# google/data-driven-discretization-1d

Hardware: AMD Instinct MI355X
Metric: grid-point-steps/s (higher is better)
Workload: dtype f32

## Files before the change

data-driven-discretization-1d_amd/csrc/capi.hip:

```cpp
#include <hip/hip_runtime.h>

#include <emmintrin.h>

#include <algorithm>
#include <chrono>
#include <cmath>
#include <condition_variable>
#include <cstdarg>
#include <cstdio>
#include <cstdlib>
#include <cstring>
#include <mutex>
#include <string>
#include <thread>
#include <type_traits>
#include <vector>

#include "../../include/ddd1d.h"
#include "dev_params.h"
#include "launch.h"
#include "launch_weno.h"
#include "ops.h"
#include "pack_weights.h"
#ifdef DDD_PROBES
// ... 235 lines not shown
  const char* name = nullptr;
};

}

struct ddd_model {
  ddd_config cfg;
  ddd::DevParams dp;
  bool mfma_ok = false;
  std::string mfma_reason;
  int kernel = DDD_KERNEL_GENERIC;
  int force_rows = 0;
  bool explicit_kernel = false;
  bool spec_folded = false;
  Plan last_plan;
  int64_t fma_per_point = 0;
  float* d_weights = nullptr;
  float* d_weights4 = nullptr;
  float* d_nullspace = nullptr;
  float* d_bias = nullptr;
  float* d_w_input = nullptr;
  float* d_w_hidden = nullptr;
  float* d_w_final4 = nullptr;
  float* d_w_final4_rt = nullptr;
  float* d_w_final4_split = nullptr;
  float* d_w_quad = nullptr;
  float* d_w_final4_half = nullptr;
  float* d_w_t16 = nullptr;
  bool wide = false;
  int tower_k = 5, tower_cb = 1;
  bool big() const { return tower_k != ddd::mfma::kKW || tower_cb != 1; }
  float4* d_frc = nullptr;
  float* d_sp = nullptr;
  float* d_trig = nullptr;
  unsigned char* d_runs = nullptr;
  bool spectral = false;
  ddd::spectral::Params sp{};
  double* d_kernels = nullptr;
  double2* d_fft_mult = nullptr;
  double2* d_fft_twiddle = nullptr;
  double* d_scratch64 = nullptr;
  size_t scratch64_doubles = 0;
  hipStream_t aux_stream[4] = {nullptr, nullptr, nullptr, nullptr};
  hipEvent_t ev_fork = nullptr, ev_join[4] = {nullptr, nullptr, nullptr, nullptr};
  struct Chain {
    bool open = false;
// ... 114 lines not shown
  in.wide = m->wide; in.tower_k = m->tower_k; in.tower_cb = m->tower_cb;
  in.no_fold = g_debug.no_fold != 0;
  in.net = net;
  const ddd::pack::Packed packed = ddd::pack::pack_weights(in);
  int rc = upload(packed.w_input, &m->d_w_input);
  if (!rc) rc = upload(packed.w_hidden, &m->d_w_hidden);
  if (!rc && packed.unsupported) rc = DDD_ERR_UNSUPPORTED;
  if (!rc) rc = upload(packed.w_final4_rt, &m->d_w_final4_rt);
  if (!rc) rc = upload(packed.w_final4, &m->d_w_final4);
  if (!rc) rc = upload(packed.w_final4_split, &m->d_w_final4_split);
  if (!rc) rc = upload(packed.w_quad, &m->d_w_quad);
  if (!rc) rc = upload(packed.w_final4_half, &m->d_w_final4_half);
  if (!rc) rc = upload(packed.w_t16, &m->d_w_t16);
  dp.w_input = m->d_w_input;
  dp.w_hidden = m->d_w_hidden;
  dp.w_final4_rt = m->d_w_final4_rt;
  dp.w_final4 = m->d_w_final4;
  dp.w_final4_split = m->d_w_final4_split;
  dp.w_quad = m->d_w_quad;
  dp.folded = packed.folded;
  dp.rt_groups = packed.rt_groups;
  dp.fin4_groups = packed.fin4_groups;
  m->spec_folded = packed.spec_folded;
  return rc;
}

bool linear_eligible(const ddd::DevParams& dp) {
  return !dp.fixed && dp.L == 1 && dp.target == ddd::TARGET_COEFFICIENTS &&
         !(dp.pao <= 0 && dp.unbiased) && dp.D <= 3 && dp.G <= ddd::kGMax && dp.K <= 7 &&
         dp.K * dp.D <= ddd::kChMax;
}

void decide_mfma(ddd_model* m) {
  const ddd::DevParams& dp = m->dp;
  char why[256] = "";
  bool ok = true;
  auto no = [&](const char* msg) { if (ok) snprintf(why, sizeof(why), "%s", msg); ok = false; };
  if (dp.N < 8 || dp.N > 256) no("num_points outside [8, 256]");
  if (dp.G > ddd::kGWide) no("stencil wider than 12");
  if (dp.G > dp.N) no("stencil wider than the grid");
  if (dp.fixed && dp.weno) no("WENO reconstruction");
  bool wide = dp.G > ddd::kGMax;
  const bool linear = linear_eligible(dp);
  if (!dp.fixed && !linear) {
    if (dp.target == ddd::TARGET_COEFFICIENTS && dp.pao <= 0 && dp.D > 2) wide = true;
    if (dp.C_out > ddd::kChMax) wide = true;
// ... 104 lines not shown

int spec_equation(const ddd_model* m, int rows) {
  const ddd::DevParams& dp = m->dp;
  if (g_debug.no_spec || m->wide || m->big()) return -1;
  if (dp.forced) {
    const int spg = rows / dp.N;
    const bool fast = spg * dp.P <= rows && dp.n_k <= 6 &&
                      spg * ddd::mfma::kTrigMax <= 3 * rows / 4 && dp.P < 256;
    if (!fast) return -1;
  }
  if (dp.fixed || dp.L != 3 || dp.act != ddd::ACT_RELU) return -1;
  if (dp.target != ddd::TARGET_COEFFICIENTS || dp.pao <= 0) return -1;
  if (dp.equation < ddd::EQ_BURGERS || dp.equation > ddd::EQ_KS_CONS) return -1;
  if (dp.D != ddd::mfma::spec_derivs(dp.equation)) return -1;
  if (dp.G != ddd::mfma::spec_stencil(dp.equation)) return -1;
  if ((dp.conservative != 0) != ddd::mfma::spec_flux_form(dp.equation)) return -1;
  int start = 0;
  for (int d = 0; d < dp.D; ++d) {
    if (dp.in_size[d] != ddd::mfma::spec_in_size(dp.equation, d) || dp.in_start[d] != start)
      return -1;
    start += dp.in_size[d];
  }
  if (m->spec_folded != ddd::mfma::spec_folded(dp.equation)) return -1;
  return dp.equation;
}

bool aligned16(const void* ptr) {
  return (reinterpret_cast<uintptr_t>(ptr) & 15u) == 0;
}

bool use_weno_kernel(const ddd_model* m) {
  return m->kernel == DDD_KERNEL_GENERIC && !m->explicit_kernel && !g_debug.no_weno &&
         ddd::weno::supports(m->dp);
}

template <int kK, int kD, typename F>
bool lean_kernel_if(int taps, int derivs, F& f) {
  if (taps != kK || derivs != kD) return false;
  f(std::integral_constant<int, kK>{}, std::integral_constant<int, kD>{});
  return true;
}
template <typename F>
bool with_lean_kernel(const ddd::DevParams& dp, F&& f) {
  if (!ddd::lean::supports(dp)) return false;
  const int t = dp.fixed ? 0 : dp.linear_taps, d = dp.D;
  return lean_kernel_if<0, 1>(t, d, f) || lean_kernel_if<0, 2>(t, d, f) ||
// ... 2238 lines not shown
    DDD_HIP(hipMalloc(reinterpret_cast<void**>(&d_in), 128 * sizeof(float)));
    DDD_HIP(hipMalloc(reinterpret_cast<void**>(&d_out), 192 * sizeof(float)));
    DDD_HIP(hipMemcpy(d_in, h_in.data(), 128 * sizeof(float), hipMemcpyHostToDevice));
    hipLaunchKernelGGL(ddd::ops::relu_clamp_probe_kernel, dim3(1), dim3(64), 0, nullptr, d_in, d_out);
    DDD_HIP(hipGetLastError());
    std::vector<float> h_out(192);
    DDD_HIP(hipMemcpy(h_out.data(), d_out, 192 * sizeof(float), hipMemcpyDeviceToHost));
    (void)hipFree(d_in);
    (void)hipFree(d_out);
    for (int l = 0; l < 64; ++l)
      for (int e = 0; e < 2; ++e) {
        const float x = h_in[2 * l + e], got = h_out[64 * e + l];
        const float want = std::isnan(x) ? 0.0f : x < 0.0f ? 0.0f : x > 1.0f ? 1.0f : x;
        if (!(got == want) || std::signbit(got))
          return fail(DDD_ERR_UNSUPPORTED,
                      "v_pk_add_f32 ... clamp is not the [0, 1] clamp the relu assumes: "
                      "input %g (element %d of pair %d) gave %g, want %g", x, e, l, got, want);
      }
    for (int l = 0; l < 64; ++l)
      if (h_out[128 + l] != (l < 32 ? (float)l : 1.0f))
        return fail(DDD_ERR_UNSUPPORTED, "constant-lane-mask select: lane %d gave %g", l,
                    h_out[128 + l]);
  }
  (void)dpp_wave_rol_ok();
  return DDD_OK;
}

}
```

data-driven-discretization-1d_amd/csrc/mfma_layout.h:

```cpp
#pragma once

#if defined(__HIP__) || defined(__HIPCC__)
#define DDD_HD __host__ __device__
#else
#define DDD_HD
#endif

namespace ddd {

constexpr int kMaxLayers = 8;
constexpr int kGMax = 8;
constexpr int kGWide = 12;
constexpr int kChMax = 16, kChWide = 24;

constexpr int kReluShift = 64;

enum : int { ACT_NONE = -1, ACT_RELU = 0, ACT_RELU6 = 1, ACT_TANH = 2,
             ACT_SOFTPLUS = 3, ACT_ELU = 4 };
enum : int { TARGET_COEFFICIENTS = 0, TARGET_SPACE_DERIVATIVES = 1,
             TARGET_TIME_DERIVATIVE = 2, TARGET_FLUX = 3 };

namespace mfma {

constexpr int kF = 32;
constexpr int kKW = 5;
constexpr int kInSteps = 3;
constexpr int kHidSteps = 81;
constexpr int kFin4K = kKW * kF + 1;
DDD_HD constexpr int flavour_stencil(bool wide) { return wide ? kGWide : kGMax; }
DDD_HD constexpr int flavour_channels(bool wide) { return wide ? kChWide : kChMax; }
constexpr int kWideDerivs = 3;
DDD_HD constexpr int flavour_net_channels(bool wide) {
  return wide ? kWideDerivs * kGWide : kChMax;
}
DDD_HD constexpr int wide_slot(int G) { return G <= kGMax ? kGMax : G; }

constexpr int kT16InSteps = 2, kT16HidSteps = 4 * kKW + 1;

DDD_HD constexpr int fin4_regs(int groups) { return (kFin4K * groups + 15) / 16; }
DDD_HD constexpr int rt_head_groups(int groups) {
  return groups % 2 == 0 ? 0 : groups == 1 ? 1 : 3;
}

constexpr int padded_rows4(int rows) { return (rows + 3) / 4 * 4; }

constexpr int kQuadHidSteps = 41, kQuadFinSteps = 41, kQuadInSteps = 2;
constexpr int kQuadRows = 2 * kQuadInSteps + 2 * kQuadHidSteps + kQuadFinSteps;

}
}
```

data-driven-discretization-1d_amd/csrc/ops.h:

```cpp
#pragma once
#include "dev_params.h"

namespace ddd {
namespace ops {

__global__ void conv1d_periodic_kernel(const float* __restrict__ in,
                                       const float* __restrict__ w,
                                       const float* __restrict__ bias,
                                       float* __restrict__ out, int batch, int n,
                                       int cin, int cout, int k, int left, int act) {
  const long total = (long)batch * n * cout;
  for (long idx = blockIdx.x * (long)blockDim.x + threadIdx.x; idx < total;
       idx += (long)gridDim.x * blockDim.x) {
    const int co = (int)(idx % cout);
    const long bx = idx / cout;
    const int x = (int)(bx % n);
    const long b = bx / n;
    float acc = 0.0f;
    for (int kk = 0; kk < k; ++kk) {
      int src = (x + kk - left) % n;
      src = src < 0 ? src + n : src;
      const float* row = in + ((size_t)b * n + src) * cin;
      const float* wk = w + (size_t)kk * cin * cout + co;
      for (int ci = 0; ci < cin; ++ci) acc = fmaf(row[ci], wk[(size_t)ci * cout], acc);
// ... 127 lines not shown
  }
}

template <int kAbid>
__device__ __forceinline__ f32x4 mfma4_bcast(float a, float b, f32x4 c) {
  return __builtin_amdgcn_mfma_f32_4x4x1f32(a, b, c, 4, kAbid, 0);
}

__global__ void mfma4_layout_probe_kernel(float* __restrict__ out) {
  const int l = threadIdx.x;
  const float a = (float)(1000 * (l >> 2) + (l & 3) + 1);
  const float b = (float)(l + 1);
#define DDD_P4(ABID)                                                        \
  {                                                                         \
    f32x4 acc = {0.5f, 0.5f, 0.5f, 0.5f};                                   \
    acc = mfma4_bcast<ABID>(a, b, acc);                                     \
    for (int r = 0; r < 4; ++r) out[(ABID * 4 + r) * 64 + l] = acc[r];      \
  }
  DDD_P4(0) DDD_P4(1) DDD_P4(2) DDD_P4(3) DDD_P4(4) DDD_P4(5) DDD_P4(6) DDD_P4(7)
  DDD_P4(8) DDD_P4(9) DDD_P4(10) DDD_P4(11) DDD_P4(12) DDD_P4(13) DDD_P4(14) DDD_P4(15)
#undef DDD_P4
}

__global__ void relu_clamp_probe_kernel(const float* __restrict__ in, float* __restrict__ out) {
  typedef float f32x2 __attribute__((ext_vector_type(2)));
  const int l = threadIdx.x;
  f32x2 v{in[2 * l], in[2 * l + 1]}, y;
  asm volatile("v_pk_add_f32 %0, %1, 0 clamp" : "=v"(y) : "v"(v));
  out[l] = y[0];
  out[64 + l] = y[1];
  float sel;
  const float x = (float)l;
  asm volatile("v_cndmask_b32_e64 %0, %1, 1.0, %2" : "=v"(sel) : "v"(x), "s"(0xffffffff00000000ull));
  out[128 + l] = sel;
}

}
}
```

data-driven-discretization-1d_amd/csrc/pack_weights.h:

```cpp
#pragma once
#include <cmath>
#include <cstddef>
#include <vector>

#include "mfma_layout.h"

namespace ddd {
namespace pack {

struct NetLayout {
  const float* weights;
  int w_off[kMaxLayers], b_off[kMaxLayers];
};

struct Input {
  int L, D, G, C_out, cout0, act, target, pao;
  const int* in_start;
  const int* in_size;
  const float (*ns8)[kGWide];
  const float (*bias8)[kGWide];
  bool wide;
  int tower_k, tower_cb;
  bool no_fold;
  NetLayout net;
};

struct Packed {
  std::vector<float> w_input, w_hidden, w_final4_rt, w_final4, w_final4_split, w_quad,
      w_final4_half, w_t16;
  int folded = 0, rt_groups = 0, fin4_groups = 0;
  bool spec_folded = false;
  bool unsupported = false;
};

inline std::vector<float> quad_rows(const float* rows64, int rows) {
  std::vector<float> out((size_t)ddd::mfma::padded_rows4(rows) * 64, 0.0f);
  for (int s = 0; s < rows; ++s)
    for (int lane = 0; lane < 64; ++lane)
      out[((size_t)(s >> 2) * 64 + lane) * 4 + (s & 3)] = rows64[(size_t)s * 64 + lane];
  return out;
}

template <class Params>
void embed_tower(const Params& dp, const std::vector<float>& wv, int tower_k,
                 int tower_c, std::vector<float>* padded, NetLayout* net) {
  const int k5 = tower_k, f32 = tower_c;
  const int shift = (k5 - 1) / 2 - dp.K / 2;
  padded->clear();
  for (int l = 0; l < dp.L; ++l) {
    const int cin = l == 0 ? 1 : f32;
    const int cout = l == dp.L - 1 ? dp.C_out : f32;
    net->w_off[l] = (int)padded->size();
// ... 112 lines not shown
        acc += (double)b_nat[start + j] * (double)in.ns8[start + j][g];
      f.b[oc] = (float)acc;
    }
  return f;
}

inline int natural_row(int k) { return k; }
inline int tile16_row(int k) { return (k / 16) * 32 + k % 16; }

inline void pack_groups4(const OutLayer& src, float up, int kc, int (*src_row)(int),
                         int first_group, int ng, float* rows) {
  for (int k = 0; k <= kc; ++k)
    for (int gi = 0; gi < ng; ++gi) {
      const int q = k * ng + gi;
      for (int r = 0; r < 4; ++r) {
        const int ch = 4 * (first_group + gi) + r;
        if (ch >= src.live) continue;
        rows[(size_t)(q / 16) * 64 + 4 * (q % 16) + r] =
            k < kc ? up * src.w[(size_t)src_row(k) * src.cols + ch] : src.b[ch];
      }
    }
}

inline std::vector<float> pack_final4_rt(const OutLayer& src, float up, int kc, int groups) {
  const auto regs = [kc](int ng) { return ((kc + 1) * ng + 15) / 16; };
  const int head = mfma::rt_head_groups(groups);
  const int total_rows = regs(head) + (groups - head) / 2 * regs(2) + regs(3);
  std::vector<float> packed((size_t)total_rows * 64, 0.0f);
  if (head > 0) pack_groups4(src, up, kc, natural_row, 0, head, packed.data());
  for (int g0 = head; g0 < groups; g0 += 2)
    pack_groups4(src, up, kc, natural_row, g0, 2,
                 packed.data() + (size_t)(regs(head) + (g0 - head) / 2 * regs(2)) * 64);
  return packed;
}


inline void pack_input16(const float* w0, const float* b0, float dn, int c0, float* rows) {
  for (int lane = 0; lane < 64; ++lane) {
    const int sg = lane >> 4, cout = c0 + (lane & 15);
    rows[lane] = dn * w0[sg * 32 + cout];
    rows[64 + lane] = sg == 0 ? dn * w0[4 * 32 + cout] : sg == 1 ? dn * b0[cout] : 0.0f;
  }
}

inline std::vector<float> pack_quad(const float* w0, const float* b0, const float* w1,
                                    const float* b1, const OutLayer& src, float dn, float up) {
// ... 63 lines not shown
    }
  }

  const float* w_nat = w(in.L - 1);
  const float* b_nat = b(in.L - 1);
  const Fold fold = fold_output_layer(in, w_nat, b_nat, kc);
  const OutLayer plain{w_nat, b_nat, in.C_out, in.C_out};

  const auto issue_cost = [](int groups) { return groups == 1 ? 13.2 : 8.1 * groups; };
  const int groups_plain = (in.C_out + 3) / 4;
  const int groups_rt_folded = ((in.D - 1) * fold.slot + in.G + 3) / 4;
  const bool fold_rt = fold.can_fold && (fold.always || issue_cost(groups_rt_folded) <=
                                                            issue_cost(groups_plain) + 2.5);
  if (fold.wide && !fold_rt) {
    out.unsupported = true;
    return out;
  }
  out.folded = fold_rt ? 1 : 0;
  out.rt_groups = fold_rt ? groups_rt_folded : groups_plain;
  const OutLayer folded_rt{fold.w.data(), fold.b.data(), fold.cols, fold.cols};
  out.w_final4_rt = pack_final4_rt(fold_rt ? folded_rt : plain, up, kc, out.rt_groups);

  const int groups_folded = (in.D * in.G + 3) / 4;
  out.spec_folded = fold.can_fold && groups_folded <= groups_plain;
  out.fin4_groups = out.spec_folded ? groups_folded : groups_plain;
  if (in.wide || big || out.fin4_groups > 4) return out;
  const OutLayer folded_spec{fold.w.data(), fold.b.data(), fold.cols, in.D * in.G};
  const OutLayer& spec = out.spec_folded ? folded_spec : plain;
  const int groups = out.fin4_groups, rows4 = mfma::fin4_regs(4), kc5 = mfma::kFin4K - 1;
  {
    std::vector<float> rows((size_t)rows4 * 64, 0.0f);
    pack_groups4(spec, up, kc5, natural_row, 0, groups, rows.data());
    out.w_final4 = quad_rows(rows.data(), rows4);
  }
  const int na = (groups + 1) / 2, chunk_rows = mfma::fin4_regs(2);
  for (int c = 0; c < 2; ++c) {
    std::vector<float> chunk((size_t)chunk_rows * 64, 0.0f);
    pack_groups4(spec, up, kc5, natural_row, c == 0 ? 0 : na, c == 0 ? na : groups - na,
                 chunk.data());
    const std::vector<float> q4 = quad_rows(chunk.data(), chunk_rows);
    out.w_final4_split.insert(out.w_final4_split.end(), q4.begin(), q4.end());
  }
  if (in.L != 3) return out;
  out.w_quad = pack_quad(w(0), b(0), w(1), b(1), spec, dn, up);
  if (in.cout0 <= 16) {
    std::vector<float> rows((size_t)rows4 * 64, 0.0f);
    pack_groups4(spec, up, 80, tile16_row, 0, groups, rows.data());
    out.w_final4_half = quad_rows(rows.data(), rows4);
    out.w_t16 = pack_t16(w(0), b(0), w(1), b(1), dn);
  }
  return out;
}

}
}
```

data-driven-discretization-1d_amd/csrc/rhs_adaptive.h:

```cpp
#pragma once
#include "rhs_mfma.h"
#include "rk23.h"
#ifdef DDD_PROBES
#include "rhs_adaptive_trace.h"
#else
#define DDD_ADAPT_TRACE_SETUP do {} while (0)
#define DDD_ADAPT_STAMP(K) do {} while (0)
#endif

namespace ddd {
namespace mfma {

template <int kRows, int kWR>
__device__ __forceinline__ double sample_sum(const DevParams& p, const Lane& ln, double v,
                                             double* red) {
  if (kRows == kWR) {
    for (int m = 1; m < p.N; m <<= 1) v += __shfl_xor(v, m, 64);
    return v;
  }
  __syncthreads();
  if constexpr (kWR == 16) {
    const int lane4 = ln.lane << 2;
    const int inner = p.N < 16 ? p.N : 16;
    for (int m = 1; m < inner; m <<= 1) {
// ... 68 lines not shown
                    sizeof(Shared<kRows, kWR, kWide>) + sizeof(AdaptiveShared<kRows>) <= 80 * 1024,
                "two 256-row workgroups per CU");
  double* red = kRows == kWR ? nullptr : reinterpret_cast<double*>(sm.un);
  const int tid = (int)threadIdx.x;
  const Lane ln = make_lane<kRows, kWR>(p, a.batch, tid, (int)blockIdx.x);
  Resident res;
  const bool fast_frc = launch_setup<kRows, kWR, kHoist, false>(p, sm, ln, a.batch, res);
  const int frc_sl = (fast_frc && tid < (kRows / p.N) * p.P)
                         ? row_sample(tid, p.inv_P) : 0;
  const bool row_live = ln.row < ln.rows_used;

  const double t0 = a.times[0];
  const double t_bound = a.times[a.n_times - 1];
  const double interval = fabs(t_bound - t0);
  const double rtol = a.rtol, atol = a.atol, max_step = a.max_step;
  const double sqrt_n = sqrt((double)p.N);
  const bool sqrt_n_pow2 = (p.N & (p.N - 1)) == 0 && (__builtin_ctz(p.N) & 1) == 0;
  const double inv_sqrt_n = 1.0 / sqrt_n;
  const size_t row_stride = (size_t)a.batch * p.N;
  const auto rms = [&](double q) {
    const double nrm = sqrt(sample_sum<kRows, kWR>(p, ln, q * q, red));
    return sqrt_n_pow2 ? nrm * inv_sqrt_n : nrm / sqrt_n;
  };
  constexpr bool kMaskedSums = kHoist && kWR == 64 && kEq >= 0 && spec_folded(kEq >= 0 ? kEq : 0);

  PackedControl* ctl = as.ctl;
  int* attempts_of = as.attempts_of;
  int* vote = as.vote;
  if (tid == 0) { vote[0] = 0; vote[1] = 0; }
  const int slot = ln.sl;
  const bool keeper = row_live && ln.pos == 0 && ln.owner;
  {
    rk23::Control c0;
    c0.init(t0, ln.valid != 0);
    if (keeper) { ctl[slot].store(c0); attempts_of[slot] = 0; }
  }
  group_barrier<kRows, kWR>();
  double y = ln.valid ? a.y0[ln.gidx] : 0.0;
  double y_new = y;
  float k0 = 0.0f, k1 = 0.0f, k2 = 0.0f;
  double te_next = 0.0;

  int phase = 0;
  int round = 0;
  bool sums_ready = false;
  DDD_ADAPT_TRACE_SETUP;
  for (;;) {
// ... 143 lines not shown
```

data-driven-discretization-1d_amd/csrc/rhs_mfma.h:

```cpp
#pragma once
#include <type_traits>
#include <utility>

#include "dev_params.h"
#include "mfma_layout.h"

namespace ddd {
namespace mfma {

constexpr int kHS = 36;
constexpr int kTrigMax = 12;
__host__ __device__ constexpr int tab_rows(bool wide) { return wide ? 4 : 4 + flavour_channels(false); }

typedef float f32x16 __attribute__((ext_vector_type(16)));
typedef float f32x4 __attribute__((ext_vector_type(4)));
typedef float f32x2 __attribute__((ext_vector_type(2)));

template <int kK_, int kCB_>
struct Tower {
  static constexpr int kK = kK_;
  static constexpr int kCB = kCB_;
  static constexpr int kC = 32 * kCB_;
  static constexpr int kHS = kC + 4;
  static constexpr int kInSteps = (kK_ + 2) / 2;
// ... 77 lines not shown
  return (eq == EQ_KS || eq == EQ_KS_CONS) ? 3 : 2;
}
__host__ __device__ constexpr bool spec_flux_form(int eq) {
  return eq == EQ_BURGERS_CONS || eq == EQ_KDV_CONS || eq == EQ_KS_CONS;
}
__host__ __device__ constexpr int spec_stencil(int eq) { return spec_flux_form(eq) ? 6 : 7; }
__host__ __device__ constexpr bool spec_forced_family(int eq) {
  return eq == EQ_BURGERS || eq == EQ_BURGERS_CONS;
}
__host__ __device__ constexpr int prio_mode(int eq) {
  return eq < 0 ? 0 : spec_forced_family(eq) ? 2 : 5;
}
__host__ __device__ constexpr int spec_in_size(int eq, int d) {
  return d == 0 ? 5
         : d == 1 ? ((eq == EQ_KDV || eq == EQ_KDV_CONS) ? 3 : 4)
         : d == 2 ? 2 : 0;
}
__host__ __device__ constexpr int spec_net_channels(int eq) {
  return spec_in_size(eq, 0) + spec_in_size(eq, 1) + (spec_derivs(eq) > 2 ? spec_in_size(eq, 2) : 0);
}
__host__ __device__ constexpr int spec_channel_deriv(int eq, int c) {
  return c < spec_in_size(eq, 0) ? 0 : c < spec_in_size(eq, 0) + spec_in_size(eq, 1) ? 1 : 2;
}
__host__ __device__ constexpr bool spec_folded(int eq) {
  return spec_derivs(eq) <= 2 &&
         (spec_derivs(eq) * spec_stencil(eq) + 3) / 4 <= (spec_net_channels(eq) + 3) / 4;
}
__host__ __device__ constexpr int spec_fin_channels(int eq) {
  return spec_folded(eq) ? spec_derivs(eq) * spec_stencil(eq) : spec_net_channels(eq);
}
__host__ __device__ constexpr int spec_fin_groups(int eq) { return (spec_fin_channels(eq) + 3) / 4; }

__device__ __forceinline__ float pick4(int s, float v0, float v1, float v2, float v3) {
  float r;
  asm("s_cmp_eq_u32 %1, 1\n\ts_cselect_b32 %0, %3, %2\n\t"
      "s_cmp_eq_u32 %1, 2\n\ts_cselect_b32 %0, %4, %0\n\t"
      "s_cmp_eq_u32 %1, 3\n\ts_cselect_b32 %0, %5, %0"
      : "=&s"(r) : "s"(s), "s"(v0), "s"(v1), "s"(v2), "s"(v3) : "scc");
  return r;
}
__device__ __forceinline__ double pick4(int s, double v0, double v1, double v2, double v3) {
  double r;
  asm("s_cmp_eq_u32 %1, 1\n\ts_cselect_b64 %0, %3, %2\n\t"
      "s_cmp_eq_u32 %1, 2\n\ts_cselect_b64 %0, %4, %0\n\t"
      "s_cmp_eq_u32 %1, 3\n\ts_cselect_b64 %0, %5, %0"
      : "=&s"(r) : "s"(s), "s"(v0), "s"(v1), "s"(v2), "s"(v3) : "scc");
  return r;
}
template <typename T, bool kSgpr = true>
// ... 832 lines not shown
                                         f32x4 (&buf)[kFin4Ahead + 1], f32x4 (&acc)[kAcc],
                                         std::integer_sequence<int, OG...>) {
  (fin4_step<NG, OG, TW, kAcc>(in, off, w, buf, acc), ...);
}

template <int NG, class TW = DefaultTower, int kAcc = NG, int kPrio = 0>
__device__ __forceinline__ void final_layer4(const float* __restrict__ in_f,
                                             const float (&w)[fin4_regs_t<TW>(NG)],
                                             const int (&off)[TW::kK], f32x4 (&acc)[kAcc]) {
  const char* __restrict__ in = reinterpret_cast<const char*>(in_f);
  constexpr int kPerTap = TW::kFinC / 4;
  f32x4 buf[kFin4Ahead + 1];
#pragma unroll
  for (int g = 0; g < kAcc; ++g) acc[g] = f32x4{0.0f, 0.0f, 0.0f, 0.0f};
#pragma unroll
  for (int og = 0; og < kFin4Ahead; ++og)
    buf[og] = *reinterpret_cast<const f32x4*>(in + off[og / kPerTap] + 16 * (og % kPerTap));
  __builtin_amdgcn_sched_group_barrier(0x100, kFin4Ahead, 0);
  if (kPrio == 5) __builtin_amdgcn_s_setprio(1);
  fin4_run<NG, TW, kAcc>(in, off, w, buf, acc, std::make_integer_sequence<int, TW::kOperandGroups>{});
  if (kPrio == 5) __builtin_amdgcn_s_setprio(3);
  fin4_mfmas<NG, (TW::kFinK - 1) * NG, fin4_regs_t<TW>(NG), kAcc>(
      w, f32x4{1.0f, 1.0f, 1.0f, 1.0f}, acc, std::make_integer_sequence<int, NG>{});
}

template <int NG, int kPrio = 0>
__device__ __forceinline__ void final_layer4_t16(const float* __restrict__ in_f,
                                                 const float (&w)[fin4_regs_t<Tile16Tower>(NG)],
                                                 const int (&off)[kKW], f32x4 (&acc)[NG]) {
  const char* __restrict__ in = reinterpret_cast<const char*>(in_f);
  f32x4 cur[4], nxt[4];
#pragma unroll
  for (int g = 0; g < NG; ++g) acc[g] = f32x4{0.0f, 0.0f, 0.0f, 0.0f};
#pragma unroll
  for (int q = 0; q < 4; ++q) cur[q] = *reinterpret_cast<const f32x4*>(in + off[0] + 16 * q);
  __builtin_amdgcn_sched_group_barrier(0x100, 4, 0);
  if (kPrio == 5) __builtin_amdgcn_s_setprio(1);
  constexpr int kNW = fin4_regs_t<Tile16Tower>(NG);
  const auto tap_steps = [&](auto tap_c) {
    constexpr int tap = decltype(tap_c)::value;
#pragma unroll
    for (int q = 0; q < 4; ++q) {
      nxt[q] = cur[q];
      if (tap + 1 < kKW) nxt[q] = *reinterpret_cast<const f32x4*>(in + off[tap + 1 < kKW ? tap + 1 : tap] + 16 * q);
    }
    fin4_mfmas<NG, (4 * tap + 0) * 4 * NG, kNW, NG>(w, f32x4{cur[0][0], cur[1][0], cur[2][0], cur[3][0]}, acc,
// ... 104 lines not shown
                                          unsigned long long* trace = nullptr) {
#define DDD_STAMP(i) do { if (kTrace && trace != nullptr && group_tid<kRows, kWR>() == 0) trace[i] = __builtin_amdgcn_s_memtime(); } while (0)
  DDD_STAMP(0);
  constexpr bool kSpec = kEq >= 0;
  const int eqn = kSpec ? kEq : p.equation;
  const int nD = kSpec ? spec_derivs(kEq) : opaque_scalar(p.D);
  const int nG = kSpec ? spec_stencil(kEq) : opaque_scalar(p.G);
  const unsigned dsel_valid = kSpec ? 0u : (unsigned)opaque_scalar((int)p.dsel_valid);
  const unsigned long long dsel_bits = kSpec ? 0ull : opaque_scalar(p.dsel_bits);
  const int rt_groups = kSpec ? 0 : opaque_scalar(p.rt_groups);
  const bool flux_form = kSpec ? spec_flux_form(kEq) : (p.conservative != 0);
  const bool fixed = kSpec ? false : (p.fixed != 0 || p.linear_taps != 0);
  const bool folded = kSpec ? spec_folded(kSpec ? kEq : 0) : (p.folded != 0);
  const int target = kSpec ? (int)TARGET_COEFFICIENTS : p.target;
  const int act = kSpec ? (int)ACT_RELU : p.act;
  const bool forced = kSpec ? (spec_forced_family(kSpec ? kEq : 0) && p.forced != 0)
                            : (p.forced != 0);
  if (kSpec) fast_forcing = true;
  const int nL = kHoist ? 3 : p.L;
  const bool pow2 = kRows == 64 || (p.N & (p.N - 1)) == 0;
  constexpr bool kOneWave = kRows == kWR;
  constexpr int kPrio = prio_mode(kEq);
  constexpr int kNG = kSpec ? spec_fin_groups(kSpec ? kEq : 0) : 2;
  constexpr int kGW = flavour_stencil(kWide);
  constexpr int kCh = flavour_net_channels(kWide);
  static_assert(!(kSpec && kWide), "the per-equation kernels have no wide flavour");
  static_assert(TW::kDefault || (!kSpec && !kWide && !kHoist && kWR == 64),
                "towers other than 5 taps x 32 channels: run-time-parameterised kernels only");
  constexpr bool kSplit = kSpec && kRows == 64 && kWR == 32 && kHoist;
  constexpr bool kQuad = kSpec && kRows == 64 && kWR == 16 && kHoist;
  static_assert(kWR != 16 || kQuad, "16-row wavefronts: per-equation integrators only");
  constexpr bool kKeepOffsets = (kWR == 64 || kSplit || kQuad) && kHoist;
  constexpr bool kKeepRows = kKeepOffsets && kEq >= 0;
  constexpr bool kKeepPatch = kKeepOffsets && !kWide;
  const int tid = opaque(group_tid<kRows, kWR>());
  const Lane ln = make_lane<kRows, kWR>(p, batch, tid, group < 0 ? (int)blockIdx.x : group);
  if (ln.owner) sm.u[ln.row] = u;
  const bool clamps_nan = !fixed && (act == ACT_RELU || act == ACT_RELU6);
  if (clamps_nan && !kOneWave) {
    if (__builtin_amdgcn_ballot_w64(u != u) != 0 && ln.lane == 0) sm.nan_flag = 1;
  }
  const auto nan_in_receptive_field = [&]() -> bool {
    const int n = p.N, lk = p.K >> 1;
    int span = p.L * (p.K - 1);
    span = span < n - 1 ? span : n - 1;
    int q = (ln.pos - p.L * lk) % n;
// ... 81 lines not shown
      } else if constexpr (!TW::kDefault) {
        group_barrier<kRows, kWR>();
        if constexpr (TW::kRolled)
          hidden_layer_rolled<TW, kWR>(p, ln, l - 1, in, out, p.N, pow2, act);
        else if (l == 1 && res.hw_valid)
          hidden_layer_stream<TW, kWR, resident_groups<TW>()>(p, ln, 0, in, out, hid_rows, act,
                                                              res.hw, res.hwb);
        else
          hidden_layer_stream<TW, kWR>(p, ln, l - 1, in, out, hid_rows, act);
      } else {
        if (!kHoist && l > 1) load_hidden(p, l - 1, ln.lane, res.hid);
        group_barrier<kRows, kWR>();
        if constexpr (TW::kTile16) {
          hidden_layer_t16<kPrio>(in, out, res.hid, res.t16_hid_off, res.t16_st_off, act);
        } else {
          hidden_layer<kWR, kKeepOffsets, kPrio>(p, ln, in, out, res.hid, hid_rows, act, res.st_off);
        }
      }
      float* tmp = in; in = out; out = tmp;
    }
    DDD_STAMP(2);
    {
      if constexpr (kQuad) {
        constexpr bool kMaskedSums = spec_folded(kSpec ? kEq : 0);
        if (frc_next) res.fk_next = forcing_phase2<kRows, kWR, kMaskedSums>(sm, res);
        group_barrier<kRows, kWR>();
        const f32x4 d4 = final_layer_quad(in, res.q_fin, res.q_fin_off);
        *reinterpret_cast<float4*>(reinterpret_cast<char*>(out) + res.q_xch_off) =
            make_float4(d4[0], d4[1], d4[2], d4[3]);
        asm volatile("s_waitcnt lgkmcnt(0)" ::: "memory");
        const float* mine = out + ln.row * kHS;
#pragma unroll
        for (int g4 = 0; g4 < kNG; ++g4) {
          const float4 v = *reinterpret_cast<const float4*>(mine + 4 * g4);
          net[4 * g4] = v.x; net[4 * g4 + 1] = v.y; net[4 * g4 + 2] = v.z; net[4 * g4 + 3] = v.w;
        }
      } else if constexpr (kSplit) {
        constexpr int kNA = (kNG + 1) / 2, kNB = kNG - kNA;
        constexpr bool kMaskedSums = spec_folded(kSpec ? kEq : 0);
        if (frc_next) res.fk_next = forcing_phase2<kRows, kWR, kMaskedSums>(sm, res);
        group_barrier<kRows, kWR>();
        int off4[kKW];
#pragma unroll
        for (int k = 0; k < kKW; ++k) off4[k] = res.fin4_off[k];
        float* xch = out + ln.lane * kHS;
        if (ln.wave == 0) {
          float wa[fin4_regs(kNA)];
#pragma unroll
          for (int s2 = 0; s2 < fin4_regs(kNA); ++s2) wa[s2] = res.w_fin4[s2];
          f32x4 acc[kNA];
          final_layer4<kNA>(in, wa, off4, acc);
#pragma unroll
          for (int g4 = 0; g4 < kNA; ++g4)
            *reinterpret_cast<float4*>(xch + 4 * g4) =
                make_float4(acc[g4][0], acc[g4][1], acc[g4][2], acc[g4][3]);
        } else if constexpr (kNB > 0) {
          float wb[fin4_regs(kNB)];
#pragma unroll
          for (int s2 = 0; s2 < fin4_regs(kNB); ++s2) wb[s2] = res.w_fin4[s2];
          f32x4 acc[kNB];
          final_layer4<kNB>(in, wb, off4, acc);
#pragma unroll
// ... 22 lines not shown
      }
      int off4[TW::kK];
      if constexpr (kKeepRows) {
#pragma unroll
        for (int s2 = 0; s2 < kFirstRows; ++s2) wf4[s2] = res.w_fin4[s2];
      }
      if constexpr (!TW::kDefault) {
        int rows_k[TW::kK];
        tap_rows_n<TW>(ln, ln.row, p.N, pow2, rows_k);
#pragma unroll
        for (int k = 0; k < TW::kK; ++k)
          off4[k] = (int)__umul24((unsigned)rows_k[k], (unsigned)(TW::kHS * 4));
      } else if constexpr (kKeepOffsets) {
#pragma unroll
        for (int k = 0; k < kKW; ++k) off4[k] = res.fin4_off[k];
      } else {
        int rows5[kKW];
        tap_rows<kRows == 64>(ln, ln.row, p.N, rows5);
#pragma unroll
        for (int k = 0; k < kKW; ++k)
          off4[k] = (int)__umul24((unsigned)rows5[k], (unsigned)(kHS * 4));
      }
      if (nL == 2) group_barrier<kRows, kWR>();
      constexpr bool kMaskedSums = kKeepRows && spec_folded(kSpec ? kEq : 0);
      if (frc_next) res.fk_next = forcing_phase2<kRows, kWR, kMaskedSums>(sm, res);
      group_barrier<kRows, kWR>();
      if constexpr (kSpec) {
        f32x4 acc4[kNG];
        if (!(ablate & 4)) {
          if constexpr (TW::kTile16) final_layer4_t16<kNG, kPrio>(in, wf4, off4, acc4);
          else final_layer4<kNG, TW, kNG, kPrio>(in, wf4, off4, acc4);
        } else {
#pragma unroll
          for (int g4 = 0; g4 < kNG; ++g4) acc4[g4] = f32x4{0.0f, 0.0f, 0.0f, 0.0f};
        }
#pragma unroll
        for (int g4 = 0; g4 < kNG; ++g4)
#pragma unroll
          for (int r4 = 0; r4 < 4; ++r4) net[4 * g4 + r4] = acc4[g4][r4];
      } else if constexpr (!kSpec) {
        constexpr int kPairRows = fin4_regs_t<TW>(2);
        const int head = rt_head_groups(rt_groups);
        int done = 0;
        if (!(ablate & 4)) {
          float wnext[kPairRows];
          const auto fetch_pair = [&](int first_group) {
            const float* __restrict__ wn = p.w_final4_rt +
                (size_t)(fin4_regs_t<TW>(head) + (first_group - head) / 2 * kPairRows) * 64 +
                opaque(ln.lane);
#pragma unroll
            for (int s2 = 0; s2 < kPairRows; ++s2) wnext[s2] = wn[s2 * 64];
          };
          if (head > 0 && head < rt_groups) fetch_pair(head);
          if (head == 3) {
// ... 775 lines not shown
```

Baseline: 4.741 billion.

## Compute lone leftover output channel with scalar FMA chain instead of MFMA group

When the network's output channel count leaves a single channel in its last group of four, the final layer now runs MFMA chains only for the full groups. The leftover channel is accumulated with a per-lane scalar FMA chain whose weights are streamed from constant memory in chunks of eight. This removes one whole 4x4 MFMA accumulator chain that would mostly compute padding. Weight packing appends the lone row, disables folding for such equations, and adds a startup probe that checks the MFMA and fmaf chains agree bit-exactly. The masked-sums predicate is split out of spec_folded so that forcing-sum behaviour is kept for those equations.

```diff
diff --git a/data-driven-discretization-1d_amd/csrc/capi.hip b/data-driven-discretization-1d_amd/csrc/capi.hip
--- a/data-driven-discretization-1d_amd/csrc/capi.hip
+++ b/data-driven-discretization-1d_amd/csrc/capi.hip
@@ -281,6 +281,7 @@
   float* d_w_input = nullptr;
   float* d_w_hidden = nullptr;
   float* d_w_final4 = nullptr;
+  bool has_lone = false;
   float* d_w_final4_rt = nullptr;
   float* d_w_final4_split = nullptr;
   float* d_w_quad = nullptr;
@@ -441,6 +442,7 @@
   dp.rt_groups = packed.rt_groups;
   dp.fin4_groups = packed.fin4_groups;
   m->spec_folded = packed.spec_folded;
+  m->has_lone = !packed.w_lone.empty();
   return rc;
 }
 
@@ -591,6 +593,7 @@
     start += dp.in_size[d];
   }
   if (m->spec_folded != ddd::mfma::spec_folded(dp.equation)) return -1;
+  if (ddd::mfma::spec_lone_channel(dp.equation) != m->has_lone) return -1;
   return dp.equation;
 }
 
@@ -2875,6 +2878,46 @@
         return fail(DDD_ERR_UNSUPPORTED, "constant-lane-mask select: lane %d gave %g", l,
                     h_out[128 + l]);
   }
+  {
+    const int steps = ddd::mfma::kFin4K;
+    std::vector<float> h_w(steps), h_b((size_t)steps * 64);
+    unsigned long long rng = 0x9e3779b97f4a7c15ull;
+    const auto uniform = [&rng]() {
+      rng = rng * 6364136223846793005ull + 1442695040888963407ull;
+      return (float)(rng >> 40) * (1.0f / 16777216.0f);
+    };
+    const float up = std::ldexp(1.0f, ddd::kReluShift), dn = std::ldexp(1.0f, -ddd::kReluShift);
+    for (int k = 0; k < steps; ++k) h_w[k] = (2.0f * uniform() - 1.0f) * up;
+    for (size_t i = 0; i < h_b.size(); ++i) {
+      const int kind = (int)(uniform() * 8.0f);
+      const float mag = kind == 0 ? 0.0f : kind == 1 ? std::ldexp(uniform(), -40)
+                        : kind == 2 ? 1.0f : uniform();
+      h_b[i] = mag * dn;
+    }
+    float *d_w = nullptr, *d_b = nullptr, *d_o = nullptr;
+    DDD_HIP(hipMalloc(reinterpret_cast<void**>(&d_w), h_w.size() * sizeof(float)));
+    DDD_HIP(hipMalloc(reinterpret_cast<void**>(&d_b), h_b.size() * sizeof(float)));
+    DDD_HIP(hipMalloc(reinterpret_cast<void**>(&d_o), 128 * sizeof(float)));
+    DDD_HIP(hipMemcpy(d_w, h_w.data(), h_w.size() * sizeof(float), hipMemcpyHostToDevice));
+    DDD_HIP(hipMemcpy(d_b, h_b.data(), h_b.size() * sizeof(float), hipMemcpyHostToDevice));
+    hipLaunchKernelGGL(ddd::ops::lone_chain_probe_kernel, dim3(1), dim3(64), 0, nullptr, d_w, d_b,
+                       steps, d_o);
+    DDD_HIP(hipGetLastError());
+    std::vector<float> h_o(128);
+    DDD_HIP(hipMemcpy(h_o.data(), d_o, h_o.size() * sizeof(float), hipMemcpyDeviceToHost));
+    (void)hipFree(d_w);
+    (void)hipFree(d_b);
+    (void)hipFree(d_o);
+    for (int l = 0; l < 64; ++l) {
+      float want = 0.0f;
+      for (int k = 0; k < steps; ++k) want = fmaf(h_w[k], h_b[(size_t)k * 64 + l], want);
+      if (std::memcmp(&h_o[l], &h_o[64 + l], sizeof(float)) != 0 ||
+          std::memcmp(&h_o[l], &want, sizeof(float)) != 0)
+        return fail(DDD_ERR_UNSUPPORTED,
+                    "lone output channel: lane %d: 4x4x1 chain %a, fmaf chain %a, host %a", l,
+                    (double)h_o[l], (double)h_o[64 + l], (double)want);
+    }
+  }
   (void)dpp_wave_rol_ok();
   return DDD_OK;
 }
diff --git a/data-driven-discretization-1d_amd/csrc/mfma_layout.h b/data-driven-discretization-1d_amd/csrc/mfma_layout.h
--- a/data-driven-discretization-1d_amd/csrc/mfma_layout.h
+++ b/data-driven-discretization-1d_amd/csrc/mfma_layout.h
@@ -43,6 +43,7 @@
 }
 
 constexpr int padded_rows4(int rows) { return (rows + 3) / 4 * 4; }
+constexpr int lone_offset() { return padded_rows4(fin4_regs(4)) * 64; }
 
 constexpr int kQuadHidSteps = 41, kQuadFinSteps = 41, kQuadInSteps = 2;
 constexpr int kQuadRows = 2 * kQuadInSteps + 2 * kQuadHidSteps + kQuadFinSteps;
diff --git a/data-driven-discretization-1d_amd/csrc/ops.h b/data-driven-discretization-1d_amd/csrc/ops.h
--- a/data-driven-discretization-1d_amd/csrc/ops.h
+++ b/data-driven-discretization-1d_amd/csrc/ops.h
@@ -173,6 +173,21 @@
 #undef DDD_P4
 }
 
+__global__ void lone_chain_probe_kernel(const float* __restrict__ w, const float* __restrict__ b,
+                                        int steps, float* __restrict__ out) {
+  const int l = threadIdx.x;
+  f32x4 acc = {0.0f, 0.0f, 0.0f, 0.0f};
+  float lone = 0.0f;
+  for (int k = 0; k < steps; ++k) {
+    const float a = w[(k + (l & 3) * 7) % steps];
+    const float bk = b[k * 64 + l];
+    acc = mfma4_bcast<0>(a, bk, acc);
+    lone = __builtin_fmaf(w[k], bk, lone);
+  }
+  out[l] = acc[0];
+  out[64 + l] = lone;
+}
+
 __global__ void relu_clamp_probe_kernel(const float* __restrict__ in, float* __restrict__ out) {
   typedef float f32x2 __attribute__((ext_vector_type(2)));
   const int l = threadIdx.x;
diff --git a/data-driven-discretization-1d_amd/csrc/pack_weights.h b/data-driven-discretization-1d_amd/csrc/pack_weights.h
--- a/data-driven-discretization-1d_amd/csrc/pack_weights.h
+++ b/data-driven-discretization-1d_amd/csrc/pack_weights.h
@@ -28,6 +28,7 @@
 struct Packed {
   std::vector<float> w_input, w_hidden, w_final4_rt, w_final4, w_final4_split, w_quad,
       w_final4_half, w_t16;
+  std::vector<float> w_lone;
   int folded = 0, rt_groups = 0, fin4_groups = 0;
   bool spec_folded = false;
   bool unsupported = false;
@@ -186,6 +187,14 @@
     }
 }
 
+inline std::vector<float> pack_lone(const OutLayer& src, float up, int kc, int (*src_row)(int),
+                                    int ch) {
+  std::vector<float> row((size_t)(kc + 1 + 15) / 16 * 16, 0.0f);
+  for (int k = 0; k < kc; ++k) row[k] = up * src.w[(size_t)src_row(k) * src.cols + ch];
+  row[kc] = src.b[ch];
+  return row;
+}
+
 inline std::vector<float> pack_final4_rt(const OutLayer& src, float up, int kc, int groups) {
   const auto regs = [kc](int ng) { return ((kc + 1) * ng + 15) / 16; };
   const int head = mfma::rt_head_groups(groups);
@@ -295,7 +304,8 @@
   out.w_final4_rt = pack_final4_rt(fold_rt ? folded_rt : plain, up, kc, out.rt_groups);
 
   const int groups_folded = (in.D * in.G + 3) / 4;
-  out.spec_folded = fold.can_fold && groups_folded <= groups_plain;
+  const bool lone = in.C_out % 4 == 1 && in.C_out > 4;
+  out.spec_folded = fold.can_fold && !lone && groups_folded <= groups_plain;
   out.fin4_groups = out.spec_folded ? groups_folded : groups_plain;
   if (in.wide || big || out.fin4_groups > 4) return out;
   const OutLayer folded_spec{fold.w.data(), fold.b.data(), fold.cols, in.D * in.G};
@@ -306,6 +316,11 @@
     pack_groups4(spec, up, kc5, natural_row, 0, groups, rows.data());
     out.w_final4 = quad_rows(rows.data(), rows4);
   }
+  if (lone && !out.spec_folded) {
+    out.w_lone = pack_lone(spec, up, kc5, natural_row, in.C_out - 1);
+    out.w_final4.insert(out.w_final4.end(), out.w_lone.begin(), out.w_lone.end());
+    out.w_final4.resize((out.w_final4.size() + 255) / 256 * 256, 0.0f);
+  }
   const int na = (groups + 1) / 2, chunk_rows = mfma::fin4_regs(2);
   for (int c = 0; c < 2; ++c) {
     std::vector<float> chunk((size_t)chunk_rows * 64, 0.0f);
diff --git a/data-driven-discretization-1d_amd/csrc/rhs_adaptive.h b/data-driven-discretization-1d_amd/csrc/rhs_adaptive.h
--- a/data-driven-discretization-1d_amd/csrc/rhs_adaptive.h
+++ b/data-driven-discretization-1d_amd/csrc/rhs_adaptive.h
@@ -114,7 +114,7 @@
     const double nrm = sqrt(sample_sum<kRows, kWR>(p, ln, q * q, red));
     return sqrt_n_pow2 ? nrm * inv_sqrt_n : nrm / sqrt_n;
   };
-  constexpr bool kMaskedSums = kHoist && kWR == 64 && kEq >= 0 && spec_folded(kEq >= 0 ? kEq : 0);
+  constexpr bool kMaskedSums = kHoist && kWR == 64 && kEq >= 0 && spec_masked_sums(kEq >= 0 ? kEq : 0);
 
   PackedControl* ctl = as.ctl;
   int* attempts_of = as.attempts_of;
diff --git a/data-driven-discretization-1d_amd/csrc/rhs_mfma.h b/data-driven-discretization-1d_amd/csrc/rhs_mfma.h
--- a/data-driven-discretization-1d_amd/csrc/rhs_mfma.h
+++ b/data-driven-discretization-1d_amd/csrc/rhs_mfma.h
@@ -123,9 +123,15 @@
 __host__ __device__ constexpr int spec_channel_deriv(int eq, int c) {
   return c < spec_in_size(eq, 0) ? 0 : c < spec_in_size(eq, 0) + spec_in_size(eq, 1) ? 1 : 2;
 }
+__host__ __device__ constexpr bool spec_lone_channel(int eq) {
+  return spec_net_channels(eq) % 4 == 1;
+}
 __host__ __device__ constexpr bool spec_folded(int eq) {
-  return spec_derivs(eq) <= 2 &&
+  return spec_derivs(eq) <= 2 && !spec_lone_channel(eq) &&
          (spec_derivs(eq) * spec_stencil(eq) + 3) / 4 <= (spec_net_channels(eq) + 3) / 4;
+}
+__host__ __device__ constexpr bool spec_masked_sums(int eq) {
+  return spec_forced_family(eq) && spec_flux_form(eq);
 }
 __host__ __device__ constexpr int spec_fin_channels(int eq) {
   return spec_folded(eq) ? spec_derivs(eq) * spec_stencil(eq) : spec_net_channels(eq);
@@ -1004,6 +1010,75 @@
   if (kPrio == 5) __builtin_amdgcn_s_setprio(3);
   fin4_mfmas<NG, (TW::kFinK - 1) * NG, fin4_regs_t<TW>(NG), kAcc>(
       w, f32x4{1.0f, 1.0f, 1.0f, 1.0f}, acc, std::make_integer_sequence<int, NG>{});
+}
+
+typedef float f32x8 __attribute__((ext_vector_type(8)));
+typedef const __attribute__((address_space(4))) f32x8* LoneChunks;
+
+template <int NGW, int K0, int NW, int... J>
+__device__ __forceinline__ void fin4_mfmas_of(const float (&w)[NW], const f32x4& b,
+                                              f32x4 (&acc)[NGW - 1],
+                                              std::integer_sequence<int, J...>) {
+  constexpr int NI = NGW - 1;
+  ((acc[J % NI] = mfma4<((K0 + J / NI) * NGW + J % NI) % 16>(
+        w[((K0 + J / NI) * NGW + J % NI) / 16], b[J / NI], acc[J % NI])), ...);
+}
+
+template <int NGW, int OG, class TW>
+__device__ __forceinline__ void fin4_lone_step(const char* __restrict__ in, const int (&off)[TW::kK],
+                                               const float (&w)[fin4_regs_t<TW>(NGW)],
+                                               f32x4 (&buf)[kFin4Ahead + 1], f32x4 (&acc)[NGW - 1],
+                                               LoneChunks wl, f32x8 (&ws)[2], float& lone) {
+  constexpr int kNext = OG + kFin4Ahead;
+  constexpr int kPerTap = TW::kFinC / 4;
+  constexpr int kChunk = OG / 2;
+  if constexpr (kNext < TW::kOperandGroups)
+    buf[kNext % (kFin4Ahead + 1)] =
+        *reinterpret_cast<const f32x4*>(in + off[kNext / kPerTap] + 16 * (kNext % kPerTap));
+  if constexpr (OG % 2 == 0) ws[(kChunk + 1) & 1] = wl[kChunk + 1];
+  const f32x4 b = buf[OG % (kFin4Ahead + 1)];
+  fin4_mfmas_of<NGW, OG * 4, fin4_regs_t<TW>(NGW)>(w, b, acc,
+                                                  std::make_integer_sequence<int, 4 * (NGW - 1)>{});
+#pragma unroll
+  for (int e = 0; e < 4; ++e) lone = __builtin_fmaf(ws[kChunk & 1][4 * (OG & 1) + e], b[e], lone);
+  if constexpr (kNext < TW::kOperandGroups) __builtin_amdgcn_sched_group_barrier(0x100, 1, 0);
+  __builtin_amdgcn_sched_group_barrier(0x008, 4 * (NGW - 1), 0);
+}
+
+template <int NGW, class TW, int... OG>
+__device__ __forceinline__ void fin4_lone_run(const char* __restrict__ in, const int (&off)[TW::kK],
+                                              const float (&w)[fin4_regs_t<TW>(NGW)],
+                                              f32x4 (&buf)[kFin4Ahead + 1], f32x4 (&acc)[NGW - 1],
+                                              LoneChunks wl, f32x8 (&ws)[2], float& lone,
+                                              std::integer_sequence<int, OG...>) {
+  (fin4_lone_step<NGW, OG, TW>(in, off, w, buf, acc, wl, ws, lone), ...);
+}
+
+template <int NGW, class TW = DefaultTower>
+__device__ __forceinline__ float final_layer4_lone(const float* __restrict__ in_f,
+                                                   const float (&w)[fin4_regs_t<TW>(NGW)],
+                                                   const float* __restrict__ w_lone,
+                                                   const int (&off)[TW::kK], f32x4 (&acc)[NGW - 1]) {
+  static_assert(NGW >= 3 && TW::kOperandGroups % 2 == 0 && (TW::kFinK - 1) % 8 == 0,
+                "two or more MFMA chains; whole chunks of eight weights, then the bias");
+  const char* __restrict__ in = reinterpret_cast<const char*>(in_f);
+  constexpr int kPerTap = TW::kFinC / 4;
+  const LoneChunks wl = (LoneChunks)w_lone;
+  f32x4 buf[kFin4Ahead + 1];
+  f32x8 ws[2];
+  ws[0] = wl[0];
+#pragma unroll
+  for (int g = 0; g < NGW - 1; ++g) acc[g] = f32x4{0.0f, 0.0f, 0.0f, 0.0f};
+#pragma unroll
+  for (int og = 0; og < kFin4Ahead; ++og)
+    buf[og] = *reinterpret_cast<const f32x4*>(in + off[og / kPerTap] + 16 * (og % kPerTap));
+  __builtin_amdgcn_sched_group_barrier(0x100, kFin4Ahead, 0);
+  float lone = 0.0f;
+  fin4_lone_run<NGW, TW>(in, off, w, buf, acc, wl, ws, lone,
+                         std::make_integer_sequence<int, TW::kOperandGroups>{});
+  fin4_mfmas_of<NGW, TW::kFinK - 1, fin4_regs_t<TW>(NGW)>(
+      w, f32x4{1.0f, 1.0f, 1.0f, 1.0f}, acc, std::make_integer_sequence<int, NGW - 1>{});
+  return __builtin_fmaf(ws[(TW::kOperandGroups / 2) & 1][0], 1.0f, lone);
 }
 
 template <int NG, int kPrio = 0>
@@ -1154,6 +1229,8 @@
   constexpr bool kOneWave = kRows == kWR;
   constexpr int kPrio = prio_mode(kEq);
   constexpr int kNG = kSpec ? spec_fin_groups(kSpec ? kEq : 0) : 2;
+  constexpr bool kLone = kSpec && spec_lone_channel(kSpec ? kEq : 0);
+  static_assert(!kLone || kPrio != 5, "final_layer4_lone carries no priority switches");
   constexpr int kGW = flavour_stencil(kWide);
   constexpr int kCh = flavour_net_channels(kWide);
   static_assert(!(kSpec && kWide), "the per-equation kernels have no wide flavour");
@@ -1281,7 +1358,7 @@
     DDD_STAMP(2);
     {
       if constexpr (kQuad) {
-        constexpr bool kMaskedSums = spec_folded(kSpec ? kEq : 0);
+        constexpr bool kMaskedSums = spec_masked_sums(kSpec ? kEq : 0);
         if (frc_next) res.fk_next = forcing_phase2<kRows, kWR, kMaskedSums>(sm, res);
         group_barrier<kRows, kWR>();
         const f32x4 d4 = final_layer_quad(in, res.q_fin, res.q_fin_off);
@@ -1296,7 +1373,7 @@
         }
       } else if constexpr (kSplit) {
         constexpr int kNA = (kNG + 1) / 2, kNB = kNG - kNA;
-        constexpr bool kMaskedSums = spec_folded(kSpec ? kEq : 0);
+        constexpr bool kMaskedSums = spec_masked_sums(kSpec ? kEq : 0);
         if (frc_next) res.fk_next = forcing_phase2<kRows, kWR, kMaskedSums>(sm, res);
         group_barrier<kRows, kWR>();
         int off4[kKW];
@@ -1365,14 +1442,23 @@
           off4[k] = (int)__umul24((unsigned)rows5[k], (unsigned)(kHS * 4));
       }
       if (nL == 2) group_barrier<kRows, kWR>();
-      constexpr bool kMaskedSums = kKeepRows && spec_folded(kSpec ? kEq : 0);
+      constexpr bool kMaskedSums = kKeepRows && spec_masked_sums(kSpec ? kEq : 0);
       if (frc_next) res.fk_next = forcing_phase2<kRows, kWR, kMaskedSums>(sm, res);
       group_barrier<kRows, kWR>();
       if constexpr (kSpec) {
         f32x4 acc4[kNG];
         if (!(ablate & 4)) {
-          if constexpr (TW::kTile16) final_layer4_t16<kNG, kPrio>(in, wf4, off4, acc4);
-          else final_layer4<kNG, TW, kNG, kPrio>(in, wf4, off4, acc4);
+          if constexpr (TW::kTile16) {
+            final_layer4_t16<kNG, kPrio>(in, wf4, off4, acc4);
+          } else if constexpr (kLone) {
+            f32x4 acc_m[kNG - 1];
+            const float lone = final_layer4_lone<kNG, TW>(in, wf4, p.w_final4 + lone_offset(), off4, acc_m);
+#pragma unroll
+            for (int g4 = 0; g4 < kNG - 1; ++g4) acc4[g4] = acc_m[g4];
+            acc4[kNG - 1] = f32x4{lone, 0.0f, 0.0f, 0.0f};
+          } else {
+            final_layer4<kNG, TW, kNG, kPrio>(in, wf4, off4, acc4);
+          }
         } else {
 #pragma unroll
           for (int g4 = 0; g4 < kNG; ++g4) acc4[g4] = f32x4{0.0f, 0.0f, 0.0f, 0.0f};
```

Result: slower. 4.473 billion (-5.6%).
